# constantingoeldel/alphabeta-rs

Hardware: AMD Instinct MI355X
Metric: ABneutral model fits/sec (pedigree x bootstraps x windows) (higher is better)
Workload: dtype f64; 1 GPU; C3: synthetic 100-edge/8-generation pedigree (N=105 rows, T=8, K=47 distinct triples), 10 starts + 10000 bootstraps per GPU (bootstraps of one window sharded over the GPUs); rows=105, windows_per_gpu=1, starts=10, bootstraps=10000, plan_device_bytes=11405122, reduction_tree=0x10040, parallelism=bootstraps sharded over 1 GPU(s), one RCCL all-gather of the bootstrap tables

## Files before the change

alphabeta_rs_amd/csrc/abn_fit_refill.hpp:

```cpp
#pragma once
#include "abn_common.hpp"
#include "abn_fit_kernel.hpp"

namespace abn {

constexpr int ST_IDLE = 13;

#ifndef ABN_REFILL_MIN_WAVES
#define ABN_REFILL_MIN_WAVES 3
#endif
template <int G, int RMAX>
__global__ __launch_bounds__(kWave, ABN_REFILL_MIN_WAVES) void abn_fit_refill_kernel(const FitArgs a) {
  static_assert(RMAX > 0, "resident mode only");
  constexpr int NG = kWave / G;
  constexpr int RR = RMAX;
  extern __shared__ __align__(16) double lds[];

  auto guard_says_stop = [&]() {
    return (__hip_atomic_load(a.guard, __ATOMIC_RELAXED, __HIP_MEMORY_SCOPE_AGENT) != 0u) == (a.guard_stop != 0);
  };
  if (a.guard && guard_says_stop()) return;
  const int lane = threadIdx.x;
  const int g = lane / G;
  const int gl = lane - g * G;
  const int dim = gl & 3;
  const unsigned total = (unsigned)((long long)a.W * a.C);
  const int N = a.N, K = a.K, TP = a.TP;

  double* pw = lds + (size_t)g * a.chain_stride;
  double* dtab = pw + kPw * TP;
  double* wconst = dtab + ((K + 1) & ~1);
  double* dobs = wconst + 4;
  uint32_t* tri_s = reinterpret_cast<uint32_t*>(dobs + ((N + 1) & ~1));

  unsigned* const pht = a.quantum > 0 ? a.park_ht + (blockIdx.x & (kParkShards - 1)) * kParkHeaderInts : nullptr;
  int* const pk = a.quantum > 0 ? a.parked + (size_t)(blockIdx.x & (kParkShards - 1)) * a.park_cap : nullptr;
  const bool canon = a.tree == kTreeCanon;
  uint32_t tidp[(RR + 1) / 2];
  for (int t = gl; t < K; t += G) tri_s[t] = a.tri[t];
#pragma unroll
  for (int q = 0; q < (RR + 1) / 2; ++q) tidp[q] = 0u;
#pragma unroll
  for (int q = 0; q < RR; ++q) {
    const int i = gl + G * q;
    if (i < N) tidp[q / 2] |= (uint32_t)a.tid[i] << (16 * (q & 1));
  }

  unsigned chain = blockIdx.x * NG + g;
  double vx[5], c[5];
  int st = ST_IDLE;
  int iter = 0, evals = 0;
  double xc = 0.0, x0 = 0.0, xr = 0.0, bx = __builtin_nan("");
  double fr = 0.0, best_cost = __builtin_inf();
  bool have_best = false;
  int fin_status = 2;
  int q_start = 0;
  bool fresh_done = false;
  bool wave_fd = false;
  bool tail_mode = false;
  bool tail_park = false;
  unsigned wstep = 0;
  unsigned gstep = 0;
#pragma unroll
  for (int k = 0; k < 5; ++k) {
    vx[k] = 0.0;
    c[k] = 0.0;
  }

  auto setup_chain = [&]() {
    const int w = (int)(chain / (unsigned)a.C);
    const int j = (int)(chain - (unsigned)w * (unsigned)a.C);
    const int wi = w * a.wstride;
    const size_t wN = (size_t)w * (size_t)N;
    if (gl == 0) {
      const double p_uu0 = a.p_uu[wi];
      wconst[0] = p_uu0;
      wconst[1] = 1.0 - p_uu0;
      wconst[2] = a.eqp[wi];
      wconst[3] = a.eqp_w[wi] * (double)N;
    }
    const uint32_t* idx_row = (a.dmode == 1) ? a.idx + (size_t)chain * (size_t)N : nullptr;
    const size_t dN = (a.dmode == 2) ? (size_t)chain * (size_t)N : wN;
#pragma unroll
    for (int q = 0; q < RR; ++q) {
      const int i = gl + G * q;
      if (i < N)
        dobs[i] = (a.dmode == 1) ? a.pred[wN + i] + a.resid[wN + idx_row[i]] : a.D[dN + i];
    }
    if (a.smode == 0) {
      const double* s0 = a.simplex0 + (size_t)chain * 20;
#pragma unroll
      for (int k = 0; k < 5; ++k) vx[k] = s0[4 * k + dim];
    } else {
      const uint32_t k0 = (uint32_t)a.seed, k1 = (uint32_t)(a.seed >> 32);
      const uint32_t wg = a.wid ? a.wid[w] : a.window_offset + (uint32_t)w, bg = a.boot_offset + (uint32_t)j;
      vx[0] = a.model[4 * w + dim];
#pragma unroll
      for (int v = 1; v < 5; ++v) {
        uint32_t r[4];
        philox4x32_10((uint32_t)(v - 1) * 2u + (uint32_t)(dim >> 1), bg, wg, kTagJitter, k0, k1, r);
        const uint32_t r0 = r[0], r1 = r[1], r2 = r[2], r3 = r[3];
        const bool odd = (dim & 1) != 0;
        vx[v] = vary_one(vx[0], odd ? r2 : r0, odd ? r3 : r1);
      }
    }
    iter = 0;
    evals = 0;
    bx = __builtin_nan("");
    best_cost = __builtin_inf();
    have_best = false;
    fin_status = 2;
    fr = 0.0;
    q_start = a.quantum > 0 ? -(int)((chain * 2654435761u >> 16) % (unsigned)a.quantum) : 0;
    st = ST_INIT0;
  };
  auto resume_chain = [&]() {
    const int w = (int)(chain / (unsigned)a.C);
    const int wi = w * a.wstride;
    const size_t wN = (size_t)w * (size_t)N;
    if (gl == 0) {
      const double p_uu0 = a.p_uu[wi];
      wconst[0] = p_uu0;
      wconst[1] = 1.0 - p_uu0;
      wconst[2] = a.eqp[wi];
      wconst[3] = a.eqp_w[wi] * (double)N;
    }
    const uint32_t* idx_row = (a.dmode == 1) ? a.idx + (size_t)chain * (size_t)N : nullptr;
    const size_t dN = (a.dmode == 2) ? (size_t)chain * (size_t)N : wN;
#pragma unroll
    for (int q = 0; q < RR; ++q) {
      const int i = gl + G * q;
      if (i < N)
        dobs[i] = (a.dmode == 1) ? a.pred[wN + i] + a.resid[wN + idx_row[i]] : a.D[dN + i];
    }
    double* sp = a.state + (size_t)chain * kStateDoubles;
    auto ld = [&](int i) { return __hip_atomic_load(sp + i, __ATOMIC_RELAXED, __HIP_MEMORY_SCOPE_AGENT); };
#pragma unroll
    for (int k = 0; k < 5; ++k) {
      vx[k] = ld(kStateSimplex + 4 * k + dim);
      c[k] = ld(kStateCosts + k);
    }
    bx = ld(kStateBest + dim);
    best_cost = ld(kStateBestCost);
    const long long ie = __double_as_longlong(ld(kStateIterEvals));
    iter = (int)(ie & 0xffffffffll);
    evals = (int)(ie >> 32);
    have_best = __double_as_longlong(ld(kStateHaveBest)) != 0;
    fin_status = 2;
    fr = 0.0;
    double acc = vx[0];
    acc = acc + vx[1];
    acc = acc + vx[2];
    acc = acc + vx[3];
    x0 = acc * (1.0 / 4.0);
    xr = x0 + (x0 - vx[4]) * 1.0;
    xc = xr;
    q_start = evals;
    st = ST_REFLECT;
  };
  if (chain < total) setup_chain();
  __syncthreads();

  auto eval = [&](double xd) -> double {
    const double al = dpp_mov<kDppQuadBcast0>(xd), be = dpp_mov<kDppQuadBcast1>(xd);
    const double wt = dpp_mov<kDppQuadBcast2>(xd), ic = dpp_mov<kDppQuadBcast3>(xd);
    const double p_mm = wconst[1];
    const double sv0 = wconst[0], sv1 = wt * p_mm, sv2 = (1.0 - wt) * p_mm;
    const double puu = p_uu_est(al, be);
    const double dq = puu - wconst[2];
    const double pen = wconst[3] * (dq * dq);
    uint32_t tr = tri_s[gl < K ? gl : 0];
    if constexpr (kMatrixFma && G == kWave) build_power_table_mx<G>(al, be, a.T, lds, a.chain_stride, dtab, lane);
    else build_power_table<G>(genmatrix(al, be), a.T, TP, pw, gl);
    __syncthreads();
#pragma unroll 1
    for (int t = gl; t < K; t += G) {
      const uint32_t trn = tri_s[t + G < K ? t + G : 0];
      dtab[t] = triple_dt(tr, pw, TP, sv0, sv1, sv2);
      tr = trn;
    }
    __syncthreads();
    double acc = 0.0;
    constexpr int RC = RR < 8 ? RR : 8;
    constexpr int NA = kWave / G;
    double av[NA];
#pragma unroll
    for (int j = 0; j < NA; ++j) av[j] = 0.0;
#pragma unroll
    for (int q0 = 0; q0 < RR; q0 += RC) {
      double dv[RC], tv[RC], x[RC];
#pragma unroll
      for (int q = 0; q < RC; ++q) {
        const int i = gl + G * (q0 + q);
        dv[q] = dobs[i < N ? i : N - 1];
        tv[q] = dtab[(tidp[(q0 + q) / 2] >> (16 * ((q0 + q) & 1))) & 0xffffu];
      }
#pragma unroll
      for (int q = 0; q < RC; ++q) {
        const double r = dv[q] - ic - tv[q];
        const double term = r * r + pen;
        x[q] = ((gl + G * (q0 + q)) < N) ? term : 0.0;
      }
      if (canon) {
#pragma unroll
        for (int q = 0; q < RC; ++q) av[(q0 + q) % NA] = av[(q0 + q) % NA] + x[q];
      } else {
#pragma unroll
        for (int q = 0; q < RC; ++q) acc = acc + x[q];
      }
    }
    acc = canon ? tree64_finish<G>(av) : group_sum_dpp<G>(acc);
    __syncthreads();
    return acc;
  };

  auto begin_iteration = [&](bool count_iter) {
    const double c_best = c[0];
    if (c_best < best_cost || (__builtin_isinf(c_best) && __builtin_isinf(best_cost) &&
                               (__builtin_signbit(c_best) == __builtin_signbit(best_cost)))) {
      bx = vx[0];
      best_cost = c_best;
      have_best = true;
    }
    if (count_iter) ++iter;
    bool converged = false;
    if (!((c[4] - c[0]) > a.gap_tol)) {
      double sum = 0.0;
#pragma unroll
      for (int k = 0; k < 5; ++k) sum = sum + c[k];
      const double c0 = sum / 5.0;
      double ss = 0.0;
#pragma unroll
      for (int k = 0; k < 5; ++k) ss = ss + (c[k] - c0) * (c[k] - c0);
      const double sd = __builtin_sqrt(1.0 / (5.0 - 1.0) * ss);
      converged = sd < a.sd_tol;
    }
    int status = -1;
    if (converged) status = 0;
    else if (iter >= a.max_iters) status = 1;
    else if (best_cost <= -__builtin_inf()) status = 3;
    bool suspend = false;
    if (a.quantum > 0 && status < 0 && evals - q_start >= a.quantum) {
      int verdict = 0;
      if (gl == 0) {
        const unsigned fq = __hip_atomic_load(a.queue, __ATOMIC_RELAXED, __HIP_MEMORY_SCOPE_AGENT);
        const int av = __hip_atomic_load(reinterpret_cast<int*>(pht) + kParkAvail, __ATOMIC_RELAXED,
                                         __HIP_MEMORY_SCOPE_AGENT);
        const unsigned tl = __hip_atomic_load(pht + kParkTail, __ATOMIC_RELAXED, __HIP_MEMORY_SCOPE_AGENT);
        verdict = ((gridDim.x * NG + fq < total || av > 0) && tl + gridDim.x * NG / kParkShards + NG < a.park_cap) ? 1 : 0;
      }
      suspend = __builtin_amdgcn_ds_bpermute(4 * (g * G), verdict) != 0;
      q_start = evals;
    }
    tail_park = false;
    if (tail_mode && status < 0 && !suspend) {
      suspend = true;
      tail_park = true;
    }
    const bool done = status >= 0 || suspend;
    fin_status = (status >= 0) ? (have_best ? status : 2) : (suspend ? kFitSuspended : fin_status);
    double acc = vx[0];
    acc = acc + vx[1];
    acc = acc + vx[2];
    acc = acc + vx[3];
    x0 = acc * (1.0 / 4.0);
    xr = x0 + (x0 - vx[4]) * 1.0;
    xc = xr;
    st = done ? ST_DONE : ST_REFLECT;
  };

#ifdef ABN_MEASUREMENT_KNOBS
  int prio_cur = 0;
#endif
  while (__ballot(st != ST_IDLE) != 0ull) {
#ifdef ABN_MEASUREMENT_KNOBS
    if (a.prio_mode != 0) {
      const int e = st != ST_IDLE ? evals : 0;
      int m = 0;
#pragma unroll
      for (int j = 0; j < NG; ++j) {
        const int ej = __builtin_amdgcn_readlane(e, j * G);
        m = ej > m ? ej : m;
      }
      int lvl = (m >= a.prio_t[0] ? 1 : 0) + (m >= a.prio_t[1] ? 1 : 0) + (m >= a.prio_t[2] ? 1 : 0);
      if (a.prio_mode == 2) lvl = 3 - lvl;
      if (lvl != prio_cur) {
        prio_cur = lvl;
        if (lvl == 0) __builtin_amdgcn_s_setprio(0);
        else if (lvl == 1) __builtin_amdgcn_s_setprio(1);
        else if (lvl == 2) __builtin_amdgcn_s_setprio(2);
        else __builtin_amdgcn_s_setprio(3);
      }
    }
#endif
    if (a.tail_cap > 0 && wave_fd && !tail_mode && (++wstep & 63u) == 0u) {
      int t = 0;
      if (lane == 0) {
        const unsigned fq = __hip_atomic_load(a.queue, __ATOMIC_RELAXED, __HIP_MEMORY_SCOPE_AGENT);
        const int av = __hip_atomic_load(reinterpret_cast<int*>(pht) + kParkAvail, __ATOMIC_RELAXED, __HIP_MEMORY_SCOPE_AGENT);
        const unsigned fin = __hip_atomic_load(a.slice_status + kSliceFinished, __ATOMIC_RELAXED, __HIP_MEMORY_SCOPE_AGENT);
        t = (gridDim.x * NG + fq >= total && av <= 0 && total - fin <= (unsigned)a.tail_cap) ? 1 : 0;
      }
      tail_mode = __builtin_amdgcn_readfirstlane(t) != 0;
    }
    const bool guard_due = a.guard_poll > 0 && (++gstep & (unsigned)(a.guard_poll - 1)) == 0u;
    int guard_stop_now = 0;
    if (guard_due && lane == 0) guard_stop_now = guard_says_stop() ? 1 : 0;
    const bool in_init = st < ST_REFLECT;
    const double f = eval(in_init ? vx[0] : xc);
    if (guard_due && __builtin_amdgcn_readfirstlane(guard_stop_now) != 0) break;
    const bool is_ref = st == ST_REFLECT, is_exp = st == ST_EXPAND, is_con = st == ST_CONTRACT;
    const bool active = is_ref || is_exp || is_con;
    const bool acc_r = is_ref && (f < c[3]) && (f >= c[0]);
    const bool go_exp = is_ref && !acc_r && (f < c[0]);
    const bool go_con = is_ref && !acc_r && !go_exp && (f >= c[3]);
    const bool nan_ref = is_ref && !acc_r && !go_exp && !go_con;
    const bool keep_r = is_exp && !(f < fr);
    const bool acc_c = is_con && (f < c[4]);
    const bool rej_c = is_con && !acc_c;
    const bool do_insert = acc_r || is_exp || acc_c;
    const bool start_shrink = nan_ref || (rej_c && a.shrink_variant != 0);
    const bool do_begin = do_insert || (rej_c && a.shrink_variant == 0);
    evals += active ? 1 : 0;
    if (rej_c && a.shrink_variant == 0 && a.no_skip == 0) {
      const int rest = a.max_iters - iter - 1;
      evals += 2 * rest;
      iter += rest;
      if (a.skipped && gl == 0 && rest > 0) atomicAdd(a.skipped, 2ull * (unsigned long long)rest);
    }
    const double xi = keep_r ? xr : xc;
    const double fi = keep_r ? fr : f;
    fr = is_ref ? f : fr;
    const double x_e = x0 + (xr - x0) * 2.0;
    const double x_c = x0 + (vx[4] - x0) * 0.5;
    xc = go_exp ? x_e : (go_con ? x_c : xc);
    st = go_exp ? ST_EXPAND : (go_con ? ST_CONTRACT : st);
    if (do_insert) {
      c[4] = fi;
      vx[4] = xi;
      insert_tail<4>(c, vx);
    }
    if (do_begin) begin_iteration(true);
    if (in_init) {
      const double tv = vx[0];
#pragma unroll
      for (int q = 0; q < 4; ++q) {
        c[q] = c[q + 1];
        vx[q] = vx[q + 1];
      }
      c[4] = f;
      vx[4] = tv;
      st = st + 1;
      if (st == ST_REFLECT) {
        evals = 5;
        sort5(c, vx);
        begin_iteration(false);
      }
    }
    if (__ballot(start_shrink) != 0ull) {
#pragma unroll 1
      for (int k = 1; k < 5; ++k) {
        const double nv = vx[0] + (vx[1] - vx[0]) * 0.5;
        const double fk = eval(start_shrink ? nv : xc);
        if (start_shrink) {
          ++evals;
#pragma unroll
          for (int q = 1; q < 4; ++q) {
            c[q] = c[q + 1];
            vx[q] = vx[q + 1];
          }
          c[4] = fk;
          vx[4] = nv;
        }
      }
      if (start_shrink) {
        sort5(c, vx);
        begin_iteration(true);
      }
    }
    if (__ballot(st == ST_DONE) != 0ull) {
      const bool fin = st == ST_DONE;
      const double b0 = dpp_mov<kDppQuadBcast0>(bx), b1 = dpp_mov<kDppQuadBcast1>(bx);
      unsigned nxt = 0xffffffffu;
      const bool parking = fin && fin_status == kFitSuspended;
      if (parking) {
        double* sp = a.state + (size_t)chain * kStateDoubles;
        auto sd = [&](int i, double v) { __hip_atomic_store(sp + i, v, __ATOMIC_RELAXED, __HIP_MEMORY_SCOPE_AGENT); };
        if (gl < 4) {
#pragma unroll
          for (int k = 0; k < 5; ++k) sd(kStateSimplex + 4 * k + gl, vx[k]);
          sd(kStateBest + gl, bx);
        }
        if (gl == 0) {
#pragma unroll
          for (int k = 0; k < 5; ++k) sd(kStateCosts + k, c[k]);
          sd(kStateBestCost, best_cost);
          sd(kStateIterEvals, __longlong_as_double((long long)(unsigned)iter | ((long long)evals << 32)));
          sd(kStateHaveBest, __longlong_as_double(have_best ? 1ll : 0ll));
        }
      } else if (fin) {
        if (gl < 4) a.best[(size_t)chain * 4 + gl] = bx;
        if (gl == 0) {
          if (a.slice_status) atomicAdd(a.slice_status + kSliceFinished, 1u);
          FitInfoDev fo;
          fo.best_cost = best_cost;
          fo.iters = iter;
          fo.evals = evals;
          fo.status = fin_status;
          fo.lanes = a.tree;
          a.info[chain] = fo;
        }
        if (a.raw) {
          double* ro = a.raw + (size_t)chain * 7;
          if (gl < 4) ro[gl] = bx;
          if (gl == 4) ro[4] = est_mm(b0, b1);
          if (gl == 5) ro[5] = est_um(b0, b1);
          if (gl == 6) ro[6] = p_uu_est(b0, b1);
        }
      }
      if (a.quantum > 0) {
        if (__ballot(parking) != 0ull) asm volatile("s_waitcnt vmcnt(0) ; abn: parked state written through" ::: "memory");
        if (parking && tail_park && gl == 0) {
          a.susp_list[atomicAdd(a.susp_count, 1)] = (int)chain;
          atomicAdd(a.slice_status + kSliceHanded, 1u);
        }
        if (parking && !tail_park && gl == 0) {
          const unsigned pos = atomicAdd(pht + kParkTail, 1u);
#ifdef ABN_MEASUREMENT_KNOBS
          if (!(a.drop_entry != 0 && pos == 0 && (blockIdx.x & (kParkShards - 1)) == 0))
#endif
          __hip_atomic_store(pk + pos, (int)chain, __ATOMIC_RELAXED, __HIP_MEMORY_SCOPE_AGENT);
          atomicAdd(reinterpret_cast<int*>(pht) + kParkAvail, 1);
        }
      }
      bool take_parked = false;
      if (fin && gl == 0) {
        if (!fresh_done) {
          const unsigned f = gridDim.x * NG + atomicAdd(a.queue, 1u);
          if (f < total) nxt = f;
          else fresh_done = true;
        }
        if (nxt == 0xffffffffu && a.quantum > 0) {
          int* avail = reinterpret_cast<int*>(pht) + kParkAvail;
          bool claimed = false;
          for (int tries = 0; tries < 1024 && !claimed; ++tries) {
            if (atomicSub(avail, 1) > 0) {
              claimed = true;
            } else {
              atomicAdd(avail, 1);
              if (__hip_atomic_load(avail, __ATOMIC_RELAXED, __HIP_MEMORY_SCOPE_AGENT) <= 0) break;
              __builtin_amdgcn_s_sleep(1);
            }
          }
          if (claimed) {
            const unsigned h = atomicAdd(pht + kParkHead, 1u);
            int cpk;
            unsigned spins = 0;
            while ((cpk = __hip_atomic_load(pk + h, __ATOMIC_RELAXED, __HIP_MEMORY_SCOPE_AGENT)) < 0 && spins < (1u << 24)) {
              __builtin_amdgcn_s_sleep(1);
              ++spins;
            }
            if (cpk >= 0) {
              nxt = (unsigned)cpk;
              take_parked = true;
            } else if (a.slice_status) {
              atomicOr(a.slice_status + kSliceError, kSliceErrLostEntry);
            }
          }
        }
      }
      nxt = (unsigned)__builtin_amdgcn_ds_bpermute(4 * (g * G), (int)nxt);
      take_parked = __builtin_amdgcn_ds_bpermute(4 * (g * G), (int)take_parked) != 0;
      fresh_done = __builtin_amdgcn_ds_bpermute(4 * (g * G), (int)fresh_done) != 0;
      wave_fd = wave_fd || (__ballot(fresh_done) != 0ull);
      if (fin) {
        st = ST_IDLE;
        if (nxt < total) {
          chain = nxt;
          if (take_parked) resume_chain();
          else setup_chain();
        }
      }
      __syncthreads();
    }
  }
}

}
```

Before: 3.386 million fits/s.

## Reload cold kernel args from kernarg segment and nest a tight hot-step loop

Rarely used kernel arguments (queue, park headers, totals, guard, state pointers) are now reloaded from the kernarg segment via opaque pointers instead of being kept live across the Nelder-Mead loop. The goal is to cut SGPR/VGPR pressure in the hot step. The step is wrapped in an inner do-while that exits only when a shrink or a finish occurs. The skipped-iteration atomic is deferred to chain completion, and tail-mode checks are gated by tail_cap at the point wave_fd is set. The cost is extra scalar loads on cold paths and more complex control flow, with a risk of subtly changed guard semantics (return instead of break).

```diff
diff --git a/alphabeta_rs_amd/csrc/abn_fit_refill.hpp b/alphabeta_rs_amd/csrc/abn_fit_refill.hpp
--- a/alphabeta_rs_amd/csrc/abn_fit_refill.hpp
+++ b/alphabeta_rs_amd/csrc/abn_fit_refill.hpp
@@ -9,6 +9,7 @@
 #ifndef ABN_REFILL_MIN_WAVES
 #define ABN_REFILL_MIN_WAVES 3
 #endif
+typedef const __attribute__((address_space(4))) FitArgs ColdArgs;
 template <int G, int RMAX>
 __global__ __launch_bounds__(kWave, ABN_REFILL_MIN_WAVES) void abn_fit_refill_kernel(const FitArgs a) {
   static_assert(RMAX > 0, "resident mode only");
@@ -16,16 +17,35 @@
   constexpr int RR = RMAX;
   extern __shared__ __align__(16) double lds[];
 
+  auto cold = [&]() {
+    ColdArgs* p = (ColdArgs*)__builtin_amdgcn_kernarg_segment_ptr();
+    asm volatile("" : "+s"(p));
+    return p;
+  };
+  auto cold_v = [](int v) {
+    asm volatile("" : "+v"(v));
+    return v;
+  };
+  auto cold_s = [](unsigned v) {
+    asm volatile("" : "+s"(v));
+    return v;
+  };
   auto guard_says_stop = [&]() {
-    return (__hip_atomic_load(a.guard, __ATOMIC_RELAXED, __HIP_MEMORY_SCOPE_AGENT) != 0u) == (a.guard_stop != 0);
+    ColdArgs* ca = cold();
+    return (__hip_atomic_load(ca->guard, __ATOMIC_RELAXED, __HIP_MEMORY_SCOPE_AGENT) != 0u) == (ca->guard_stop != 0);
   };
   if (a.guard && guard_says_stop()) return;
   const int lane = threadIdx.x;
   const int g = lane / G;
   const int gl = lane - g * G;
-  const int dim = gl & 3;
-  const unsigned total = (unsigned)((long long)a.W * a.C);
   const int N = a.N, K = a.K, TP = a.TP;
+  auto total_of = [](ColdArgs* ca) { return (unsigned)((long long)ca->W * ca->C); };
+  const int grid_v = cold_v((int)gridDim.x), block_v = cold_v((int)blockIdx.x);
+  const int max_iters_v = cold_v(a.max_iters), quantum_v = cold_v(a.quantum);
+  const int guard_mask = a.guard_poll - 1;
+  auto slots = [&]() { return (unsigned)__builtin_amdgcn_readfirstlane(grid_v) * NG; };
+  auto shard_of = [&]() { return (unsigned)__builtin_amdgcn_readfirstlane(block_v) & (kParkShards - 1); };
+  auto park_header = [&](ColdArgs* ca) { return ca->park_ht + shard_of() * kParkHeaderInts; };
 
   double* pw = lds + (size_t)g * a.chain_stride;
   double* dtab = pw + kPw * TP;
@@ -33,8 +53,6 @@
   double* dobs = wconst + 4;
   uint32_t* tri_s = reinterpret_cast<uint32_t*>(dobs + ((N + 1) & ~1));
 
-  unsigned* const pht = a.quantum > 0 ? a.park_ht + (blockIdx.x & (kParkShards - 1)) * kParkHeaderInts : nullptr;
-  int* const pk = a.quantum > 0 ? a.parked + (size_t)(blockIdx.x & (kParkShards - 1)) * a.park_cap : nullptr;
   const bool canon = a.tree == kTreeCanon;
   uint32_t tidp[(RR + 1) / 2];
   for (int t = gl; t < K; t += G) tri_s[t] = a.tri[t];
@@ -59,6 +77,7 @@
   bool wave_fd = false;
   bool tail_mode = false;
   bool tail_park = false;
+  int skip_rest = 0;
   unsigned wstep = 0;
   unsigned gstep = 0;
 #pragma unroll
@@ -67,40 +86,48 @@
     c[k] = 0.0;
   }
 
-  auto setup_chain = [&]() {
-    const int w = (int)(chain / (unsigned)a.C);
-    const int j = (int)(chain - (unsigned)w * (unsigned)a.C);
-    const int wi = w * a.wstride;
+  auto load_observations = [&](ColdArgs* ca, int w, int cgl) {
+    const int wi = w * ca->wstride;
     const size_t wN = (size_t)w * (size_t)N;
-    if (gl == 0) {
-      const double p_uu0 = a.p_uu[wi];
+    if (cgl == 0) {
+      const double p_uu0 = ca->p_uu[wi];
       wconst[0] = p_uu0;
       wconst[1] = 1.0 - p_uu0;
-      wconst[2] = a.eqp[wi];
-      wconst[3] = a.eqp_w[wi] * (double)N;
-    }
-    const uint32_t* idx_row = (a.dmode == 1) ? a.idx + (size_t)chain * (size_t)N : nullptr;
-    const size_t dN = (a.dmode == 2) ? (size_t)chain * (size_t)N : wN;
+      wconst[2] = ca->eqp[wi];
+      wconst[3] = ca->eqp_w[wi] * (double)N;
+    }
+    const int dmode = ca->dmode;
+    const uint32_t* idx_row = (dmode == 1) ? ca->idx + (size_t)chain * (size_t)N : nullptr;
+    const size_t dN = (dmode == 2) ? (size_t)chain * (size_t)N : wN;
 #pragma unroll
     for (int q = 0; q < RR; ++q) {
-      const int i = gl + G * q;
+      const int i = cgl + G * q;
       if (i < N)
-        dobs[i] = (a.dmode == 1) ? a.pred[wN + i] + a.resid[wN + idx_row[i]] : a.D[dN + i];
-    }
-    if (a.smode == 0) {
-      const double* s0 = a.simplex0 + (size_t)chain * 20;
-#pragma unroll
-      for (int k = 0; k < 5; ++k) vx[k] = s0[4 * k + dim];
+        dobs[i] = (dmode == 1) ? ca->pred[wN + i] + ca->resid[wN + idx_row[i]] : ca->D[dN + i];
+    }
+  };
+  auto setup_chain = [&]() {
+    ColdArgs* ca = cold();
+    const int cgl = cold_v(gl), cdim = cgl & 3;
+    const int w = (int)(chain / (unsigned)ca->C);
+    const int j = (int)(chain - (unsigned)w * (unsigned)ca->C);
+    load_observations(ca, w, cgl);
+    if (ca->smode == 0) {
+      const double* s0 = ca->simplex0 + (size_t)chain * 20;
+#pragma unroll
+      for (int k = 0; k < 5; ++k) vx[k] = s0[4 * k + cdim];
     } else {
-      const uint32_t k0 = (uint32_t)a.seed, k1 = (uint32_t)(a.seed >> 32);
-      const uint32_t wg = a.wid ? a.wid[w] : a.window_offset + (uint32_t)w, bg = a.boot_offset + (uint32_t)j;
-      vx[0] = a.model[4 * w + dim];
+      const uint64_t seed = ca->seed;
+      const uint32_t k0 = (uint32_t)seed, k1 = (uint32_t)(seed >> 32);
+      const uint32_t* const wid = ca->wid;
+      const uint32_t wg = wid ? wid[w] : ca->window_offset + (uint32_t)w, bg = ca->boot_offset + (uint32_t)j;
+      vx[0] = ca->model[4 * w + cdim];
 #pragma unroll
       for (int v = 1; v < 5; ++v) {
         uint32_t r[4];
-        philox4x32_10((uint32_t)(v - 1) * 2u + (uint32_t)(dim >> 1), bg, wg, kTagJitter, k0, k1, r);
+        philox4x32_10((uint32_t)(v - 1) * 2u + (uint32_t)(cdim >> 1), bg, wg, kTagJitter, k0, k1, r);
         const uint32_t r0 = r[0], r1 = r[1], r2 = r[2], r3 = r[3];
-        const bool odd = (dim & 1) != 0;
+        const bool odd = (cdim & 1) != 0;
         vx[v] = vary_one(vx[0], odd ? r2 : r0, odd ? r3 : r1);
       }
     }
@@ -111,36 +138,22 @@
     have_best = false;
     fin_status = 2;
     fr = 0.0;
-    q_start = a.quantum > 0 ? -(int)((chain * 2654435761u >> 16) % (unsigned)a.quantum) : 0;
+    const int quantum = ca->quantum;
+    q_start = quantum > 0 ? -(int)((chain * 2654435761u >> 16) % (unsigned)quantum) : 0;
     st = ST_INIT0;
   };
   auto resume_chain = [&]() {
-    const int w = (int)(chain / (unsigned)a.C);
-    const int wi = w * a.wstride;
-    const size_t wN = (size_t)w * (size_t)N;
-    if (gl == 0) {
-      const double p_uu0 = a.p_uu[wi];
-      wconst[0] = p_uu0;
-      wconst[1] = 1.0 - p_uu0;
-      wconst[2] = a.eqp[wi];
-      wconst[3] = a.eqp_w[wi] * (double)N;
-    }
-    const uint32_t* idx_row = (a.dmode == 1) ? a.idx + (size_t)chain * (size_t)N : nullptr;
-    const size_t dN = (a.dmode == 2) ? (size_t)chain * (size_t)N : wN;
-#pragma unroll
-    for (int q = 0; q < RR; ++q) {
-      const int i = gl + G * q;
-      if (i < N)
-        dobs[i] = (a.dmode == 1) ? a.pred[wN + i] + a.resid[wN + idx_row[i]] : a.D[dN + i];
-    }
-    double* sp = a.state + (size_t)chain * kStateDoubles;
+    ColdArgs* ca = cold();
+    const int cgl = cold_v(gl), cdim = cgl & 3;
+    load_observations(ca, (int)(chain / (unsigned)ca->C), cgl);
+    double* sp = ca->state + (size_t)chain * kStateDoubles;
     auto ld = [&](int i) { return __hip_atomic_load(sp + i, __ATOMIC_RELAXED, __HIP_MEMORY_SCOPE_AGENT); };
 #pragma unroll
     for (int k = 0; k < 5; ++k) {
-      vx[k] = ld(kStateSimplex + 4 * k + dim);
+      vx[k] = ld(kStateSimplex + 4 * k + cdim);
       c[k] = ld(kStateCosts + k);
     }
-    bx = ld(kStateBest + dim);
+    bx = ld(kStateBest + cdim);
     best_cost = ld(kStateBestCost);
     const long long ie = __double_as_longlong(ld(kStateIterEvals));
     iter = (int)(ie & 0xffffffffll);
@@ -158,7 +171,7 @@
     q_start = evals;
     st = ST_REFLECT;
   };
-  if (chain < total) setup_chain();
+  if (chain < total_of(cold())) setup_chain();
   __syncthreads();
 
   auto eval = [&](double xd) -> double {
@@ -170,8 +183,9 @@
     const double dq = puu - wconst[2];
     const double pen = wconst[3] * (dq * dq);
     uint32_t tr = tri_s[gl < K ? gl : 0];
-    if constexpr (kMatrixFma && G == kWave) build_power_table_mx<G>(al, be, a.T, lds, a.chain_stride, dtab, lane);
-    else build_power_table<G>(genmatrix(al, be), a.T, TP, pw, gl);
+    const int T = (int)cold_s((unsigned)a.T);
+    if constexpr (kMatrixFma && G == kWave) build_power_table_mx<G>(al, be, T, lds, a.chain_stride, dtab, lane);
+    else build_power_table<G>(genmatrix(al, be), T, TP, pw, gl);
     __syncthreads();
 #pragma unroll 1
     for (int t = gl; t < K; t += G) {
@@ -237,17 +251,20 @@
     }
     int status = -1;
     if (converged) status = 0;
-    else if (iter >= a.max_iters) status = 1;
+    else if (iter >= max_iters_v) status = 1;
     else if (best_cost <= -__builtin_inf()) status = 3;
     bool suspend = false;
-    if (a.quantum > 0 && status < 0 && evals - q_start >= a.quantum) {
+    if (quantum_v > 0 && status < 0 && evals - q_start >= quantum_v) {
       int verdict = 0;
-      if (gl == 0) {
-        const unsigned fq = __hip_atomic_load(a.queue, __ATOMIC_RELAXED, __HIP_MEMORY_SCOPE_AGENT);
+      if (cold_v(gl) == 0) {
+        ColdArgs* ca = cold();
+        unsigned* const pht = park_header(ca);
+        const unsigned fq = __hip_atomic_load(ca->queue, __ATOMIC_RELAXED, __HIP_MEMORY_SCOPE_AGENT);
         const int av = __hip_atomic_load(reinterpret_cast<int*>(pht) + kParkAvail, __ATOMIC_RELAXED,
                                          __HIP_MEMORY_SCOPE_AGENT);
         const unsigned tl = __hip_atomic_load(pht + kParkTail, __ATOMIC_RELAXED, __HIP_MEMORY_SCOPE_AGENT);
-        verdict = ((gridDim.x * NG + fq < total || av > 0) && tl + gridDim.x * NG / kParkShards + NG < a.park_cap) ? 1 : 0;
+        const unsigned ns = slots();
+        verdict = ((ns + fq < total_of(ca) || av > 0) && tl + ns / kParkShards + NG < ca->park_cap) ? 1 : 0;
       }
       suspend = __builtin_amdgcn_ds_bpermute(4 * (g * G), verdict) != 0;
       q_start = evals;
@@ -273,90 +290,101 @@
   int prio_cur = 0;
 #endif
   while (__ballot(st != ST_IDLE) != 0ull) {
+    bool start_shrink;
+    do {
+      asm volatile("; abn: hot step begin");
 #ifdef ABN_MEASUREMENT_KNOBS
-    if (a.prio_mode != 0) {
-      const int e = st != ST_IDLE ? evals : 0;
-      int m = 0;
-#pragma unroll
-      for (int j = 0; j < NG; ++j) {
-        const int ej = __builtin_amdgcn_readlane(e, j * G);
-        m = ej > m ? ej : m;
-      }
-      int lvl = (m >= a.prio_t[0] ? 1 : 0) + (m >= a.prio_t[1] ? 1 : 0) + (m >= a.prio_t[2] ? 1 : 0);
-      if (a.prio_mode == 2) lvl = 3 - lvl;
-      if (lvl != prio_cur) {
-        prio_cur = lvl;
-        if (lvl == 0) __builtin_amdgcn_s_setprio(0);
-        else if (lvl == 1) __builtin_amdgcn_s_setprio(1);
-        else if (lvl == 2) __builtin_amdgcn_s_setprio(2);
-        else __builtin_amdgcn_s_setprio(3);
-      }
-    }
+      if (a.prio_mode != 0) {
+        const int e = st != ST_IDLE ? evals : 0;
+        int m = 0;
+#pragma unroll
+        for (int j = 0; j < NG; ++j) {
+          const int ej = __builtin_amdgcn_readlane(e, j * G);
+          m = ej > m ? ej : m;
+        }
+        int lvl = (m >= a.prio_t[0] ? 1 : 0) + (m >= a.prio_t[1] ? 1 : 0) + (m >= a.prio_t[2] ? 1 : 0);
+        if (a.prio_mode == 2) lvl = 3 - lvl;
+        if (lvl != prio_cur) {
+          prio_cur = lvl;
+          if (lvl == 0) __builtin_amdgcn_s_setprio(0);
+          else if (lvl == 1) __builtin_amdgcn_s_setprio(1);
+          else if (lvl == 2) __builtin_amdgcn_s_setprio(2);
+          else __builtin_amdgcn_s_setprio(3);
+        }
+      }
 #endif
-    if (a.tail_cap > 0 && wave_fd && !tail_mode && (++wstep & 63u) == 0u) {
-      int t = 0;
-      if (lane == 0) {
-        const unsigned fq = __hip_atomic_load(a.queue, __ATOMIC_RELAXED, __HIP_MEMORY_SCOPE_AGENT);
-        const int av = __hip_atomic_load(reinterpret_cast<int*>(pht) + kParkAvail, __ATOMIC_RELAXED, __HIP_MEMORY_SCOPE_AGENT);
-        const unsigned fin = __hip_atomic_load(a.slice_status + kSliceFinished, __ATOMIC_RELAXED, __HIP_MEMORY_SCOPE_AGENT);
-        t = (gridDim.x * NG + fq >= total && av <= 0 && total - fin <= (unsigned)a.tail_cap) ? 1 : 0;
-      }
-      tail_mode = __builtin_amdgcn_readfirstlane(t) != 0;
-    }
-    const bool guard_due = a.guard_poll > 0 && (++gstep & (unsigned)(a.guard_poll - 1)) == 0u;
-    int guard_stop_now = 0;
-    if (guard_due && lane == 0) guard_stop_now = guard_says_stop() ? 1 : 0;
-    const bool in_init = st < ST_REFLECT;
-    const double f = eval(in_init ? vx[0] : xc);
-    if (guard_due && __builtin_amdgcn_readfirstlane(guard_stop_now) != 0) break;
-    const bool is_ref = st == ST_REFLECT, is_exp = st == ST_EXPAND, is_con = st == ST_CONTRACT;
-    const bool active = is_ref || is_exp || is_con;
-    const bool acc_r = is_ref && (f < c[3]) && (f >= c[0]);
-    const bool go_exp = is_ref && !acc_r && (f < c[0]);
-    const bool go_con = is_ref && !acc_r && !go_exp && (f >= c[3]);
-    const bool nan_ref = is_ref && !acc_r && !go_exp && !go_con;
-    const bool keep_r = is_exp && !(f < fr);
-    const bool acc_c = is_con && (f < c[4]);
-    const bool rej_c = is_con && !acc_c;
-    const bool do_insert = acc_r || is_exp || acc_c;
-    const bool start_shrink = nan_ref || (rej_c && a.shrink_variant != 0);
-    const bool do_begin = do_insert || (rej_c && a.shrink_variant == 0);
-    evals += active ? 1 : 0;
-    if (rej_c && a.shrink_variant == 0 && a.no_skip == 0) {
-      const int rest = a.max_iters - iter - 1;
-      evals += 2 * rest;
-      iter += rest;
-      if (a.skipped && gl == 0 && rest > 0) atomicAdd(a.skipped, 2ull * (unsigned long long)rest);
-    }
-    const double xi = keep_r ? xr : xc;
-    const double fi = keep_r ? fr : f;
-    fr = is_ref ? f : fr;
-    const double x_e = x0 + (xr - x0) * 2.0;
-    const double x_c = x0 + (vx[4] - x0) * 0.5;
-    xc = go_exp ? x_e : (go_con ? x_c : xc);
-    st = go_exp ? ST_EXPAND : (go_con ? ST_CONTRACT : st);
-    if (do_insert) {
-      c[4] = fi;
-      vx[4] = xi;
-      insert_tail<4>(c, vx);
-    }
-    if (do_begin) begin_iteration(true);
-    if (in_init) {
-      const double tv = vx[0];
-#pragma unroll
-      for (int q = 0; q < 4; ++q) {
-        c[q] = c[q + 1];
-        vx[q] = vx[q + 1];
-      }
-      c[4] = f;
-      vx[4] = tv;
-      st = st + 1;
-      if (st == ST_REFLECT) {
-        evals = 5;
-        sort5(c, vx);
-        begin_iteration(false);
-      }
-    }
+      if (wave_fd && !tail_mode && (++wstep & 63u) == 0u) {
+        int t = 0;
+        if (cold_v(lane) == 0) {
+          ColdArgs* ca = cold();
+          const unsigned total = total_of(ca);
+          const unsigned fq = __hip_atomic_load(ca->queue, __ATOMIC_RELAXED, __HIP_MEMORY_SCOPE_AGENT);
+          const int av = __hip_atomic_load(reinterpret_cast<int*>(park_header(ca)) + kParkAvail, __ATOMIC_RELAXED, __HIP_MEMORY_SCOPE_AGENT);
+          const unsigned fin = __hip_atomic_load(ca->slice_status + kSliceFinished, __ATOMIC_RELAXED, __HIP_MEMORY_SCOPE_AGENT);
+          t = (slots() + fq >= total && av <= 0 && total - fin <= (unsigned)ca->tail_cap) ? 1 : 0;
+        }
+        tail_mode = __builtin_amdgcn_readfirstlane(t) != 0;
+      }
+      const int gmask = (int)cold_s((unsigned)guard_mask);
+      const bool guard_due = gmask >= 0 && (++gstep & (unsigned)gmask) == 0u;
+      int guard_stop_now = 0;
+      if (guard_due) {
+        if (cold_v(lane) == 0) guard_stop_now = guard_says_stop() ? 1 : 0;
+      }
+      const bool in_init = st < ST_REFLECT;
+      const double f = eval(in_init ? vx[0] : xc);
+      if (guard_due && __builtin_amdgcn_readfirstlane(guard_stop_now) != 0) return;
+      const bool is_ref = st == ST_REFLECT, is_exp = st == ST_EXPAND, is_con = st == ST_CONTRACT;
+      const bool active = is_ref || is_exp || is_con;
+      const bool acc_r = is_ref && (f < c[3]) && (f >= c[0]);
+      const bool go_exp = is_ref && !acc_r && (f < c[0]);
+      const bool go_con = is_ref && !acc_r && !go_exp && (f >= c[3]);
+      const bool nan_ref = is_ref && !acc_r && !go_exp && !go_con;
+      const bool keep_r = is_exp && !(f < fr);
+      const bool acc_c = is_con && (f < c[4]);
+      const bool rej_c = is_con && !acc_c;
+      const bool do_insert = acc_r || is_exp || acc_c;
+      const int shrink_variant = (int)cold_s((unsigned)a.shrink_variant);
+      start_shrink = nan_ref || (rej_c && shrink_variant != 0);
+      const bool do_begin = do_insert || (rej_c && shrink_variant == 0);
+      evals += active ? 1 : 0;
+      if (rej_c && shrink_variant == 0 && (int)cold_s((unsigned)a.no_skip) == 0) {
+        const int rest = cold()->max_iters - iter - 1;
+        evals += 2 * rest;
+        iter += rest;
+        skip_rest = rest;
+      }
+      const double xi = keep_r ? xr : xc;
+      const double fi = keep_r ? fr : f;
+      fr = is_ref ? f : fr;
+      const double x_e = x0 + (xr - x0) * 2.0;
+      const double x_c = x0 + (vx[4] - x0) * 0.5;
+      xc = go_exp ? x_e : (go_con ? x_c : xc);
+      st = go_exp ? ST_EXPAND : (go_con ? ST_CONTRACT : st);
+      if (do_insert) {
+        c[4] = fi;
+        vx[4] = xi;
+        insert_tail<4>(c, vx);
+      }
+      if (do_begin) begin_iteration(true);
+      if (in_init) {
+        const double tv = vx[0];
+#pragma unroll
+        for (int q = 0; q < 4; ++q) {
+          c[q] = c[q + 1];
+          vx[q] = vx[q + 1];
+        }
+        c[4] = f;
+        vx[4] = tv;
+        st = st + 1;
+        if (st == ST_REFLECT) {
+          evals = 5;
+          sort5(c, vx);
+          begin_iteration(false);
+        }
+      }
+      asm volatile("; abn: hot step end");
+    } while (__ballot(start_shrink || st == ST_DONE) == 0ull);
     if (__ballot(start_shrink) != 0ull) {
 #pragma unroll 1
       for (int k = 1; k < 5; ++k) {
@@ -379,19 +407,26 @@
       }
     }
     if (__ballot(st == ST_DONE) != 0ull) {
+      ColdArgs* ca = cold();
+      const int cgl = cold_v(gl);
+      const unsigned total = total_of(ca);
+      const int quantum = ca->quantum;
+      const unsigned shard = shard_of();
+      unsigned* const pht = quantum > 0 ? ca->park_ht + shard * kParkHeaderInts : nullptr;
+      int* const pk = quantum > 0 ? ca->parked + (size_t)shard * ca->park_cap : nullptr;
       const bool fin = st == ST_DONE;
       const double b0 = dpp_mov<kDppQuadBcast0>(bx), b1 = dpp_mov<kDppQuadBcast1>(bx);
       unsigned nxt = 0xffffffffu;
       const bool parking = fin && fin_status == kFitSuspended;
       if (parking) {
-        double* sp = a.state + (size_t)chain * kStateDoubles;
+        double* sp = ca->state + (size_t)chain * kStateDoubles;
         auto sd = [&](int i, double v) { __hip_atomic_store(sp + i, v, __ATOMIC_RELAXED, __HIP_MEMORY_SCOPE_AGENT); };
-        if (gl < 4) {
-#pragma unroll
-          for (int k = 0; k < 5; ++k) sd(kStateSimplex + 4 * k + gl, vx[k]);
-          sd(kStateBest + gl, bx);
-        }
-        if (gl == 0) {
+        if (cgl < 4) {
+#pragma unroll
+          for (int k = 0; k < 5; ++k) sd(kStateSimplex + 4 * k + cgl, vx[k]);
+          sd(kStateBest + cgl, bx);
+        }
+        if (cgl == 0) {
 #pragma unroll
           for (int k = 0; k < 5; ++k) sd(kStateCosts + k, c[k]);
           sd(kStateBestCost, best_cost);
@@ -399,48 +434,52 @@
           sd(kStateHaveBest, __longlong_as_double(have_best ? 1ll : 0ll));
         }
       } else if (fin) {
-        if (gl < 4) a.best[(size_t)chain * 4 + gl] = bx;
-        if (gl == 0) {
-          if (a.slice_status) atomicAdd(a.slice_status + kSliceFinished, 1u);
+        if (cgl < 4) ca->best[(size_t)chain * 4 + cgl] = bx;
+        if (cgl == 0) {
+          unsigned long long* const skipped = ca->skipped;
+          if (skipped && skip_rest > 0) atomicAdd(skipped, 2ull * (unsigned long long)skip_rest);
+          unsigned* const slice_status = ca->slice_status;
+          if (slice_status) atomicAdd(slice_status + kSliceFinished, 1u);
           FitInfoDev fo;
           fo.best_cost = best_cost;
           fo.iters = iter;
           fo.evals = evals;
           fo.status = fin_status;
-          fo.lanes = a.tree;
-          a.info[chain] = fo;
-        }
-        if (a.raw) {
-          double* ro = a.raw + (size_t)chain * 7;
-          if (gl < 4) ro[gl] = bx;
-          if (gl == 4) ro[4] = est_mm(b0, b1);
-          if (gl == 5) ro[5] = est_um(b0, b1);
-          if (gl == 6) ro[6] = p_uu_est(b0, b1);
-        }
-      }
-      if (a.quantum > 0) {
+          fo.lanes = ca->tree;
+          ca->info[chain] = fo;
+        }
+        double* const raw = ca->raw;
+        if (raw) {
+          double* ro = raw + (size_t)chain * 7;
+          if (cgl < 4) ro[cgl] = bx;
+          if (cgl == 4) ro[4] = est_mm(b0, b1);
+          if (cgl == 5) ro[5] = est_um(b0, b1);
+          if (cgl == 6) ro[6] = p_uu_est(b0, b1);
+        }
+      }
+      if (quantum > 0) {
         if (__ballot(parking) != 0ull) asm volatile("s_waitcnt vmcnt(0) ; abn: parked state written through" ::: "memory");
-        if (parking && tail_park && gl == 0) {
-          a.susp_list[atomicAdd(a.susp_count, 1)] = (int)chain;
-          atomicAdd(a.slice_status + kSliceHanded, 1u);
-        }
-        if (parking && !tail_park && gl == 0) {
+        if (parking && tail_park && cgl == 0) {
+          ca->susp_list[atomicAdd(ca->susp_count, 1)] = (int)chain;
+          atomicAdd(ca->slice_status + kSliceHanded, 1u);
+        }
+        if (parking && !tail_park && cgl == 0) {
           const unsigned pos = atomicAdd(pht + kParkTail, 1u);
 #ifdef ABN_MEASUREMENT_KNOBS
-          if (!(a.drop_entry != 0 && pos == 0 && (blockIdx.x & (kParkShards - 1)) == 0))
+          if (!(ca->drop_entry != 0 && pos == 0 && shard == 0))
 #endif
           __hip_atomic_store(pk + pos, (int)chain, __ATOMIC_RELAXED, __HIP_MEMORY_SCOPE_AGENT);
           atomicAdd(reinterpret_cast<int*>(pht) + kParkAvail, 1);
         }
       }
       bool take_parked = false;
-      if (fin && gl == 0) {
+      if (fin && cgl == 0) {
         if (!fresh_done) {
-          const unsigned f = gridDim.x * NG + atomicAdd(a.queue, 1u);
+          const unsigned f = slots() + atomicAdd(ca->queue, 1u);
           if (f < total) nxt = f;
           else fresh_done = true;
         }
-        if (nxt == 0xffffffffu && a.quantum > 0) {
+        if (nxt == 0xffffffffu && quantum > 0) {
           int* avail = reinterpret_cast<int*>(pht) + kParkAvail;
           bool claimed = false;
           for (int tries = 0; tries < 1024 && !claimed; ++tries) {
@@ -463,8 +502,8 @@
             if (cpk >= 0) {
               nxt = (unsigned)cpk;
               take_parked = true;
-            } else if (a.slice_status) {
-              atomicOr(a.slice_status + kSliceError, kSliceErrLostEntry);
+            } else if (ca->slice_status) {
+              atomicOr(ca->slice_status + kSliceError, kSliceErrLostEntry);
             }
           }
         }
@@ -472,9 +511,10 @@
       nxt = (unsigned)__builtin_amdgcn_ds_bpermute(4 * (g * G), (int)nxt);
       take_parked = __builtin_amdgcn_ds_bpermute(4 * (g * G), (int)take_parked) != 0;
       fresh_done = __builtin_amdgcn_ds_bpermute(4 * (g * G), (int)fresh_done) != 0;
-      wave_fd = wave_fd || (__ballot(fresh_done) != 0ull);
+      wave_fd = wave_fd || (__ballot(fresh_done) != 0ull && ca->tail_cap > 0);
       if (fin) {
         st = ST_IDLE;
+        skip_rest = 0;
         if (nxt < total) {
           chain = nxt;
           if (take_parked) resume_chain();
```

Result: faster. 3.539 million fits/s, median of 6 (+4.5%).
